# Ignalina/znippy

Hardware: AMD Instinct MI355X
Metric: decompress MB/s (uncompressed) + compress MB/s, 100k x 10KB archive (higher is better)
Workload: dtype u8; 1 GPU; 100k x 10KiB text chunks (BASELINE configs[1]); rows_per_gpu=100000, chunk_bytes=10240, bytes_per_gpu=1024000000, blob_bytes_per_gpu=6400000, parallelism=row-cursor ranges x1, pipelining=step k+1 queued before step k's counters are read (two runs in flight)

## Files before the change

### znippy_amd/csrc/api.hip

```cpp
#include <unistd.h>
#include "common.h"
#include "encode.h"
#include "../../include/znippy_hip.h"
#include "host/enc_plan.h"
#include "host/gz_plan.h"
#include "host/range_plan.h"
#include "host/rows_plan.h"
#include "host/run_overlap.h"

#include <algorithm>
#include <cstdio>
#include <cstdlib>
#include <cstring>
#include <chrono>
#include <memory>
#include <new>
#include <stdexcept>
#include <string>
#include <vector>
#include <unordered_map>

namespace zn {
int measure_b3_pass_ns(int cus, hipStream_t s, float *ns_per_pass_per_simd, float *ghz);
size_t decode_lit_scratch_bytes(int grid);
// ... 64 lines not shown
    uint8_t *enc_prov = nullptr;
    size_t enc_prov_cap = 0;
    uint32_t *enc_seq = nullptr;
    EncTables *enc_tabs = nullptr;
    hipStream_t aux = nullptr;
    hipStream_t copy = nullptr;
    uint8_t *lit_scratch_b = nullptr;
    uint8_t *fz_lit_pool = nullptr;
    unsigned long long *fz_seq_pool = nullptr;
    uint64_t fz_lit_cap = 0, fz_seq_cap = 0;
    uint16_t *bx_fse_pool = nullptr;
    uint16_t *bx_huf_pool = nullptr;
    uint64_t bx_fse_cap = 0, bx_huf_cap = 0;
    uint32_t *rx_pool = nullptr, *rx_chunk = nullptr;
    uint8_t *rx_cdone = nullptr;
    uint64_t rx_cap = 0;
    uint8_t *vs_pool = nullptr;
    uint64_t vs_cap = 0;
    uint8_t *rr_pool[2] = {nullptr, nullptr};
    uint64_t rr_cap[2] = {0, 0};
    hipEvent_t ev_fork = nullptr, ev_join = nullptr, ev_join2 = nullptr;
    std::vector<KTime> ktimes;
    int n_ktimes = 0;
    std::vector<hipEvent_t> event_pool;
    bool ktime_open = false;
    std::vector<std::pair<size_t, void *>> pinned_pool;
    size_t pinned_pool_bytes = 0;
    std::vector<std::pair<size_t, void *>> dev_pool;
    std::unordered_map<void *, size_t> dev_sizes;
    size_t dev_pool_bytes = 0;
    struct : RowsSwitches {
        unsigned lds_pad = 0;
        int store_g = 0;
        bool edbg = false, no_fused_store = false, no_fork_verify = false, no_run_lanes = false, nohash = false, fz_only = false, tdbg = false, no_fuse_hash = false, trace = false, no_pack = false;
        int ktime = 2;
        bool poison = false;
        int poison_byte = 0;
    } sw;
    int poison_hold = 0;
    int cus = 256;
    bool fork_verify = false;
    hipStream_t lane = nullptr;
    hipEvent_t ev_mark = nullptr, lane_join = nullptr;
    hipEvent_t lane_ev[2][2] = {{nullptr, nullptr}, {nullptr, nullptr}};
    unsigned lane_n[2] = {0, 0};
    bool lanes_on = false, main_dirty = true, mark_pending = false;
    struct LaneRun { zn_run_desc d; hipEvent_t ev; bool on_lane, valid; } lane_prev = {}, lane_hist[2][2] = {};
    uint64_t lane_stats[5] = {0, 0, 0, 0, 0};
    int live_tables = 0;
    bool closing = false;
    unsigned long long *clk_buf = nullptr;
    enum Diag { DIAG_FUSED, DIAG_ITEMS, DIAG_FZ, DIAG_GENERAL, DIAG_BX, DIAG_ENCODE, DIAG_N };
    unsigned long long *diag[DIAG_N] = {};
};

static void read_switches(znippy_ctx *ctx) {
    auto on = [](const char *n) { const char *v = getenv(n); return v && *v && *v != '0'; };
    if (const char *e = getenv("ZNIPPY_DBG")) ctx->sw.dbg = atoi(e);
    if (const char *e = getenv("ZNIPPY_LDS_PAD")) ctx->sw.lds_pad = (unsigned)atoi(e);
    ctx->sw.no_block_items = on("ZNIPPY_NO_BLOCK_ITEMS");
    ctx->sw.no_fused_blocks = on("ZNIPPY_NO_FUSED_BLOCKS");
    ctx->sw.ddbg = on("ZNIPPY_DDBG");
    ctx->sw.edbg = on("ZNIPPY_EDBG");
    ctx->sw.no_fused_store = on("ZNIPPY_NO_FUSED_STORE");
    ctx->sw.nohash = on("ZNIPPY_NOHASH");
    ctx->sw.no_roles = on("ZNIPPY_NO_ROLES");
    ctx->sw.no_fz = on("ZNIPPY_NO_FZ");
    ctx->sw.tdbg = on("ZNIPPY_TDBG");
    ctx->sw.trace = on("ZNIPPY_TRACE");
    ctx->sw.no_lean = on("ZNIPPY_NO_LEAN");
    ctx->sw.no_fork_verify = on("ZNIPPY_NO_FORK_VERIFY");
    ctx->sw.no_run_lanes = on("ZNIPPY_NO_RUN_LANES");
    ctx->sw.no_pack = on("ZNIPPY_NO_PACK");
    if (const char *e = getenv("ZNIPPY_STORE_G")) ctx->sw.store_g = atoi(e) == 1 ? 1 : (atoi(e) == 2 ? 2 : 0);
    ctx->sw.no_stored_only = on("ZNIPPY_NO_STORED_ONLY");
    ctx->sw.no_rx = on("ZNIPPY_NO_RX");
    ctx->sw.no_fuse_hash = on("ZNIPPY_NO_FUSE_HASH");
    ctx->sw.no_bx = on("ZNIPPY_NO_BX");
    if (const char *e = getenv("ZNIPPY_BX_BIG")) { ctx->sw.bx_big = (unsigned)atoi(e); ctx->sw.bx_big_set = true; }
    if (const char *lv = getenv("ZNIPPY_LEVEL")) { const int v = atoi(lv); if (v >= 1 && v <= 22) ctx->level = v; }
    if (const char *wl = getenv("ZNIPPY_WINDOW_LOG")) { const int v = atoi(wl); if (v == 0 || (v >= WINDOW_LOG_MIN && v <= WINDOW_LOG_MAX)) ctx->window_log = v; }
    if (const char *gc = getenv("ZNIPPY_GZ_CUT")) {
        char *end = nullptr;
        const unsigned long long v = strtoull(gc, &end, 10);
        if (*gc >= '0' && *gc <= '9' && end && !*end && gzcut::cut_valid(v)) ctx->gz_cut = v;
    }
    if (const char *bc = getenv("ZNIPPY_BX_CHECKSUM")) { const int v = atoi(bc); if (v == 0 || v == 1) ctx->batch_checksums = v; }
    if (const char *gs = getenv("ZNIPPY_GEN_SHARE")) { const int v = atoi(gs); if (v >= 1 && v <= 4) ctx->gen_share = v; }
    ctx->sw.fz_only = on("ZNIPPY_FZ_ONLY");
    if (const char *e = getenv("ZNIPPY_ROLES_MIN")) ctx->sw.roles_min = (unsigned)atoi(e);
    if (const char *e = getenv("ZNIPPY_KTIME")) ctx->sw.ktime = atoi(e);
    if (const char *e = getenv("ZNIPPY_POISON")) {
        char *end = nullptr;
        const long v = strtol(e, &end, e[0] == '0' && (e[1] == 'x' || e[1] == 'X') ? 16 : 10);
        if (*e && end && !*end && v >= 0 && v <= 255) { ctx->sw.poison = true; ctx->sw.poison_byte = (int)v; }
    }
}

static hipError_t poison_dev(znippy_ctx *ctx, void *p, size_t bytes) {
    if (!p || !bytes) return hipSuccess;
    const hipError_t e = hipMemsetAsync(p, ctx->sw.poison_byte, bytes, ctx->stream);
    return e != hipSuccess ? e : hipStreamSynchronize(ctx->stream);
}

static void *pinned_take(znippy_ctx *ctx, size_t bytes, size_t *cap) {
    size_t best = ctx->pinned_pool.size();
    for (size_t i = 0; i < ctx->pinned_pool.size(); i++)
        if (ctx->pinned_pool[i].first >= bytes && ctx->pinned_pool[i].first <= 4 * bytes + 4096 &&
            (best == ctx->pinned_pool.size() || ctx->pinned_pool[i].first < ctx->pinned_pool[best].first))
// ... 2388 lines not shown
    }
    if (!r->d_ldm) {
        std::vector<uint64_t> desc(r->n, LDM_NONE);
        for (const LdmRound &e : r->h_ldm) desc[e.round] = e.desc;
        LdmRound *dl = nullptr;
        uint64_t *dd = nullptr;
        if (tmalloc(ctx, &dl, sizeof(LdmRound) * r->h_ldm.size()) != hipSuccess || tmalloc(ctx, &dd, 8 * (size_t)r->n) != hipSuccess ||
            hipMemcpy(dl, r->h_ldm.data(), sizeof(LdmRound) * r->h_ldm.size(), hipMemcpyHostToDevice) != hipSuccess ||
            hipMemcpy(dd, desc.data(), 8 * (size_t)r->n, hipMemcpyHostToDevice) != hipSuccess) {
            (void)hipGetLastError();
            tfree(ctx, dl);
            tfree(ctx, dd);
            return false;
        }
        r->d_ldm = dl; r->d_ldm_desc = dd;
    }
    return true;
}

struct EncRun { const void *d_src; void *d_blob_out; uint64_t blob_cap; unsigned slot; ResSlab res; uint32_t *tree_out; uint32_t align; const uint32_t *pad; };
static_assert(ENC_HIGH_TIER_LEVEL == HIGH_TIER_LEVEL, "host/enc_plan.h restates the tier boundary of encode.h");

static EncShape rounds_shape(const znippy_rounds *r) {
    return EncShape{r->n, r->n_items, r->n_small, r->n_wide, r->in_bytes, r->enc_bytes, r->fuse_tiles, r->plan.n_tiles, r->n_tree_entries, r->ldm_entries,
                    r->store_incompressible, r->emit_tree, r->blob_align};
}
static EncodeArgs rounds_encode_args(znippy_ctx *ctx, const znippy_rounds *r, const EncPlan &p, const EncRun &run) {
    EncodeArgs a{};
    a.items = r->items;
    a.src = (const uint8_t *)run.d_src; a.src_off = r->src_off; a.len = r->len;
    a.prov = ctx->enc_prov; a.seq_scratch = ctx->enc_seq;
    a.piece_len = r->piece_len; a.piece_start = r->piece_start; a.tabs = ctx->enc_tabs;
    a.high = p.high;
    a.tail_mark = p.tail_mark;
    a.window_log = p.window_log;
    if (p.far) { a.ldm = ctx->ldm; a.ldm_desc = r->d_ldm_desc; }
    if (ctx->sw.edbg)
        a.dbg = diag_cycle<8>(ctx, znippy_ctx::DIAG_ENCODE, ctx->stream, nullptr, [](const unsigned long long *h) {
            if (h[0]) fprintf(stderr, "[znippy edbg] wide blocks=%llu  cycles per block: setup=%.0f matching=%.0f literals=%.0f sequences=%.0f\n", h[0],
                              (double)h[1] / h[0], (double)h[2] / h[0], (double)h[3] / h[0], (double)h[4] / h[0]);
        });
    return a;
}
static GatherArgs rounds_gather_args(znippy_ctx *ctx, const znippy_rounds *r, const EncPlan &p, const EncRun &run) {
    GatherArgs g{};
    g.items = r->items; g.n_pieces = r->n_items; g.piece_len = r->piece_len; g.piece_start = r->piece_start;
    g.local_excl = r->local_excl; g.block_tot = r->block_tot; g.prov = ctx->enc_prov;
    g.src = (const uint8_t *)run.d_src; g.src_off = r->src_off;
    g.blob_out = (uint8_t *)run.d_blob_out; g.blob_cap = run.blob_cap;
    g.blob_offset = run.res.blob_offset(); g.blob_size = run.res.blob_size(); g.total = run.res.total(); g.overflow = run.res.overflow();
    g.stored = p.store_decide ? r->stored : nullptr;
    g.skip_stored_copy = p.fuse_store ? 1 : 0;
    g.pad = run.pad;
    g.small_pieces = p.small_pieces ? 1 : 0;
    return g;
}

static int enc_clear(znippy_ctx *ctx, znippy_rounds *r, const EncPlan &, const EncRun &run) {
    hipStream_t s = ctx->stream;
    if (r->run_seq >= 2) HIPCHK(ctx, hipStreamWaitEvent(s, r->ev_res[run.slot], 0));
    HIPCHK(ctx, hipMemsetAsync(run.res.base, 0, ResSlab::clear_bytes(r->n), s));
    HIPCHK(ctx, hipMemsetAsync(ctx->cursor, 0, 64, s));
    HIPCHK(ctx, hipEventRecord(ctx->ev_fork, s));
    return ZNIPPY_OK;
}

static int enc_far_index(znippy_ctx *ctx, znippy_rounds *r, const EncPlan &p, const EncRun &run) {
    if (!p.far) return ZNIPPY_OK;
    ktime_begin(ctx, "ldm_index");
    HIPCHK(ctx, hipMemsetAsync(ctx->ldm, 0xFF, 4 * r->ldm_entries, ctx->stream));
    launch_ldm_index(r->d_ldm, (uint32_t)r->h_ldm.size(), r->ldm_chunks, (const uint8_t *)run.d_src, r->src_off, r->len, ctx->ldm, ctx->stream);
    ktime_end(ctx);
    return ZNIPPY_OK;
// ... 46 lines not shown
}

static void enc_gather(znippy_ctx *ctx, znippy_rounds *r, const EncPlan &p, const EncRun &run) {
    const GatherArgs g = rounds_gather_args(ctx, r, p, run);
    timed(ctx, "gather", ctx->stream, [&] { launch_gather(g, ctx->stream); });
}

static int enc_hash_store(znippy_ctx *ctx, znippy_rounds *r, const EncPlan &p, const EncRun &run) {
    if (p.fuse_store) return hash_rounds_async(ctx, r, run.res, run.d_src, nullptr, run.d_blob_out, run.blob_cap, run.align, run.tree_out);
    if (p.fork_aux) HIPCHK(ctx, hipStreamWaitEvent(ctx->stream, ctx->ev_join, 0));
    return ZNIPPY_OK;
}

static int enc_results_out(znippy_ctx *ctx, znippy_rounds *r, const EncPlan &, const EncRun &run) {
    HIPCHK(ctx, hipEventRecord(r->ev_enc[run.slot], ctx->stream));
    HIPCHK(ctx, hipStreamWaitEvent(ctx->copy, r->ev_enc[run.slot], 0));
    const uint32_t n16 = (uint32_t)((r->res_bytes + 15) / 16);
    hipLaunchKernelGGL(k_results_out, dim3(std::min<uint32_t>((n16 + 255) / 256, 8)), dim3(256), 0, ctx->copy,
                       reinterpret_cast<uint4 *>(r->h_res_m[run.slot]), reinterpret_cast<const uint4 *>(run.res.base), n16);
    if (run.tree_out) {
        const uint32_t t16 = 2 * r->n_tree_entries;
        hipLaunchKernelGGL(k_results_out, dim3(std::min<uint32_t>((t16 + 255) / 256, 8)), dim3(256), 0, ctx->copy,
                           reinterpret_cast<uint4 *>(r->h_tree_m[run.slot]), reinterpret_cast<const uint4 *>(run.tree_out), t16);
    }
    HIPCHK(ctx, hipEventRecord(r->ev_res[run.slot], ctx->copy));
    return ZNIPPY_OK;
}

static int rounds_launch(znippy_ctx *ctx, znippy_rounds *r, const void *d_src, void *d_blob_out, uint64_t blob_cap, unsigned slot, bool *queued) {
    ctx->n_ktimes = 0;
    if (!r->n) return ZNIPPY_OK;
    int rc = ensure_encoder(ctx);
    if (rc) return rc;
    EncEnv env{ctx->level, ctx->window_log, ctx->encode_grid, ctx->encode_grid_small, (bool)ctx->sw.nohash, (bool)ctx->sw.no_fuse_hash, (bool)ctx->sw.no_fused_store, false};
    env.ldm_ok = enc_window_log(env) && ensure_ldm(ctx, r);
    if (r->prov_bytes + 64 > ctx->enc_prov_cap) {
        HIPCHK(ctx, hipStreamSynchronize(ctx->stream));
        if (ctx->enc_prov) (void)hipFree(ctx->enc_prov);
        ctx->enc_prov = nullptr; ctx->enc_prov_cap = 0;
        HIPCHK(ctx, hipMalloc(&ctx->enc_prov, r->prov_bytes + 64));
        ctx->enc_prov_cap = r->prov_bytes + 64;
        if (ctx->sw.poison) HIPCHK(ctx, poison_dev(ctx, ctx->enc_prov, ctx->enc_prov_cap));
    }
    const EncPlan p = enc_plan(rounds_shape(r), env);
    const EncRun run{d_src, d_blob_out, blob_cap, slot, r->dev(slot), p.tree_out ? r->tree_m[slot] : nullptr, r->blob_align, p.pad ? r->piece_pad : nullptr};
    *queued = true;
    if ((rc = enc_clear(ctx, r, p, run)) || (rc = enc_far_index(ctx, r, p, run))) return rc;
    enc_blocks(ctx, r, p, run);
    if ((rc = enc_hash_beside(ctx, r, p, run))) return rc;
    enc_layout(ctx, r, p, run);
    enc_gather(ctx, r, p, run);
    if ((rc = enc_hash_store(ctx, r, p, run)) || (rc = enc_results_out(ctx, r, p, run))) return rc;
    HIPCHK(ctx, hipGetLastError());
    r->tree_run[slot] = p.emit_tree;
    r->slot = slot;
    r->run_seq++;
    return ZNIPPY_OK;
}

static void rounds_abandon(znippy_ctx *ctx, znippy_rounds *r, unsigned slot) {
    if (hipEventRecord(ctx->ev_join, ctx->aux) == hipSuccess) (void)hipStreamWaitEvent(ctx->stream, ctx->ev_join, 0);
    (void)hipStreamWaitEvent(ctx->copy, r->ev_enc[slot], 0);
    (void)hipStreamSynchronize(ctx->stream);
    (void)hipStreamSynchronize(ctx->copy);
    (void)hipGetLastError();
}
static int rounds_queue(znippy_ctx *ctx, znippy_rounds *r, const void *d_src, void *d_blob_out, uint64_t blob_cap) {
// ... 997 lines not shown
```

### znippy_amd/csrc/encode.h

```cpp
#pragma once
#include "common.h"
#include <cstring>
#include <vector>

namespace zn {

constexpr uint32_t BLOCK_BYTES = 128 * 1024;
constexpr uint32_t HDR_ROOM = 16;
constexpr uint32_t MAX_SEQ = 16384;
constexpr uint32_t SKIP_PIECE = 64u << 10;

struct FseSymTT {
    int32_t delta_find_state;
    uint32_t delta_nb_bits;
};

struct EncTables {
    uint16_t ll_state[64], ml_state[64], of_state[32];
    FseSymTT ll_tt[36], ml_tt[53], of_tt[29];
};

constexpr uint32_t ITEM_SKIP = 1, ITEM_FIRST = 2;

struct EncItem {
    uint32_t round;
    uint32_t block;
    uint32_t n_blocks;
    uint32_t flags;
    uint64_t prov;
};

__host__ __device__ inline uint64_t enc_slot_bytes(uint32_t n) { return ((HDR_ROOM + 16 + 2ull * n + (n >> 2) + 64) + 15) & ~15ull; }

struct EncodeArgs {
    const EncItem *items;
    const uint32_t *order;
    uint32_t n_items;
    const uint32_t *n_items_dev;
    unsigned long long *dbg;
    uint32_t *retry_list, *retry_count;
    uint32_t *cursor;
    uint32_t batch;
    const uint8_t *src;
    const uint64_t *src_off, *len;
    uint8_t *prov;
    uint32_t *seq_scratch;
    uint32_t *piece_len;
    uint64_t *piece_start;
    const EncTables *tabs;
    int tail_mark;
    int high;
    int fuse_tiles;
    HashArgs h;
    int window_log;
    const uint32_t *ldm;
    const uint64_t *ldm_desc;
};

constexpr uint64_t LDM_NONE = 0;
constexpr uint32_t LDM_MIN_LOG = 11, LDM_MAX_LOG = 22;
constexpr uint64_t LDM_MAX_ENTRIES = 1ull << 27;
constexpr uint32_t LDM_CHUNK = 16384;
constexpr int WINDOW_LOG_MIN = 17, WINDOW_LOG_MAX = 27;
struct LdmRound {
    uint32_t round;
    uint32_t first_chunk;
    uint64_t desc;
};
__host__ __device__ inline uint32_t ldm_log2(uint64_t len) {
    uint32_t l = LDM_MIN_LOG;
    while (l < LDM_MAX_LOG && (1ull << l) * 64 < len) l++;
    return l;
}

struct GatherArgs {
    const EncItem *items;
    uint32_t n_pieces;
    const uint32_t *piece_len;
    const uint64_t *piece_start;
    const uint64_t *local_excl, *block_tot;
    const uint8_t *prov, *src;
    const uint64_t *src_off;
    uint8_t *blob_out;
    uint64_t blob_cap;
// ... 22 lines not shown
```

### znippy_amd/csrc/host/enc_plan.cc

```cpp
#include "enc_plan.h"

#include <algorithm>

int enc_window_log(const EncEnv &e) {
    return e.level >= ENC_HIGH_TIER_LEVEL ? e.window_log : 0;
}

static EncLaunch enc_share(const EncShape &s, uint32_t n_items, int g) {
    EncLaunch l{};
    l.on = n_items != 0;
    if (!l.on) return l;
    l.n_items = n_items;
    l.use_order = !(n_items == s.n_items);
    l.batch = std::max<uint32_t>(1, std::min<uint32_t>(16, n_items / (uint32_t)(g * 2)));
    l.grid = std::min<int>(g, (int)n_items);
    return l;
}

EncPlan enc_plan(const EncShape &s, const EncEnv &e) {
    EncPlan p{};
    p.high = e.level >= ENC_HIGH_TIER_LEVEL;
    p.window_log = enc_window_log(e);
    p.tail_mark = p.high && !p.window_log;
    p.far = p.window_log && s.ldm_entries && e.ldm_ok;
    p.store_decide = s.store_incompressible;
    p.pad = s.blob_align > 1;
    p.emit_tree = s.emit_tree && !e.nohash;
    p.tree_out = p.emit_tree && s.n_tree_entries;
    p.fuse_hash = s.fuse_tiles && !s.store_incompressible && !e.nohash && !e.no_fuse_hash;
    const bool heavy = s.in_bytes && (s.in_bytes - s.enc_bytes) * 2 >= s.in_bytes;
    p.fuse_store = heavy && !s.store_incompressible &&
                   !e.no_fused_store && !e.nohash;
    p.fork_aux = !p.fuse_store && !p.fuse_hash;
    p.hash_beside = p.fork_aux && !e.nohash;
    p.small_pieces = s.n_items && s.n_wide == 0 && (p.fuse_store || s.in_bytes / s.n_items <= 16384);
    p.wide = enc_share(s, s.n_wide, e.encode_grid);
    p.small = enc_share(s, s.n_small, e.encode_grid_small);
    if (p.small.on && p.fuse_hash)
        p.small.grid = std::min<int>(e.encode_grid_small, (int)((s.plan_n_tiles + s.fuse_tiles - 1) / s.fuse_tiles));
    if (s.n_small) {
        p.retry.on = true;
        p.retry.n_items = s.n_small; p.retry.use_order = true;
        p.retry.batch = 1;
        p.retry.grid = std::min<int>(e.encode_grid, (int)s.n_small);
    }
    return p;
}
```

### znippy_amd/csrc/host/enc_plan.h

```cpp
#pragma once
#include <stddef.h>
#include <stdint.h>

constexpr int ENC_HIGH_TIER_LEVEL = 4;

struct EncShape {
    uint32_t n;
    uint32_t n_items;
    uint32_t n_small, n_wide;
    uint64_t in_bytes, enc_bytes;
    int fuse_tiles;
    uint32_t plan_n_tiles;
    uint32_t n_tree_entries;
    uint64_t ldm_entries;
    bool store_incompressible;
    bool emit_tree;
    uint32_t blob_align;
};

struct EncEnv {
    int level, window_log;
    int encode_grid, encode_grid_small;
    bool nohash, no_fuse_hash, no_fused_store;
    bool ldm_ok;
};

struct EncLaunch {
    bool on;
    uint32_t n_items;
    bool use_order;
    int grid;
    uint32_t batch;
};

struct EncPlan {
    bool high;
    int window_log;
    bool tail_mark;
    bool far;
    bool fuse_hash;
    bool fuse_store;
    bool fork_aux;
    bool hash_beside;
    bool emit_tree;
    bool tree_out;
    bool store_decide;
    bool pad;
    bool small_pieces;
    EncLaunch wide, small, retry;
};

int enc_window_log(const EncEnv &e);
EncPlan enc_plan(const EncShape &s, const EncEnv &e);

struct ResSlab {
    uint8_t *base;
    uint32_t n;
    uint64_t *total() const { return reinterpret_cast<uint64_t *>(base); }
    uint32_t *overflow() const { return reinterpret_cast<uint32_t *>(base + 8); }
    uint64_t *blob_offset() const { return reinterpret_cast<uint64_t *>(base + 16); }
    uint64_t *blob_size() const { return blob_offset() + n; }
    uint32_t *digests() const { return reinterpret_cast<uint32_t *>(base + 16 + 16 * (size_t)n); }
    static size_t clear_bytes(size_t n) { return 16 + 16 * n; }
    static size_t bytes(size_t n) { return 16 + n * (8 + 8 + 32); }
};
```

### znippy_amd/csrc/zstd_encode.hip

```cpp
#include "common.h"
#include "encode.h"
#include "hash_dev.h"

namespace zn {


__device__ __forceinline__ uint32_t ld32(const uint8_t *p) {
    uint32_t v;
    __builtin_memcpy(&v, p, 4);
    return v;
}
__device__ __forceinline__ uint4 ld128(const uint8_t *p) {
    uint4 v;
    __builtin_memcpy(&v, p, 16);
    return v;
}
template <uint32_t HASH_LOG>
__device__ __forceinline__ uint32_t hash4(uint32_t v) { return (v * 2654435761u) >> (32 - HASH_LOG); }
__device__ __forceinline__ int hib(uint32_t v) { return 31 - __clz(v); }

__device__ __forceinline__ bool ldm_anchor(uint32_t v) { return (hash4<22>(v) & 63u) == 0; }
__device__ __forceinline__ uint32_t ldm_key(const uint8_t *p) {
    uint64_t h = 0;
#pragma unroll
// ... 48 lines not shown
        add(1, 1);
        while (n > 0) {
            *p++ = (uint8_t)acc;
            acc >>= 8;
            n = n > 8 ? n - 8 : 0;
        }
        return p;
    }
};

struct CState {
    uint32_t v;
    const uint16_t *st;
    const FseSymTT *tt;
    uint32_t log;
    __device__ __forceinline__ void init(const uint16_t *st_, const FseSymTT *tt_, uint32_t log_, uint32_t sym) {
        st = st_; tt = tt_; log = log_;
        const FseSymTT t = tt[sym];
        uint32_t nb = (t.delta_nb_bits + (1u << 15)) >> 16;
        uint32_t val = (nb << 16) - t.delta_nb_bits;
        v = st[(int32_t)(val >> nb) + t.delta_find_state];
    }
    __device__ __forceinline__ void encode(BitW &b, uint32_t sym) {
        const FseSymTT t = tt[sym];
        uint32_t nb = (v + t.delta_nb_bits) >> 16;
        b.add(v, nb);
        v = st[(int32_t)(v >> nb) + t.delta_find_state];
    }
    __device__ __forceinline__ void flush(BitW &b) { b.add(v, log); }
};

constexpr uint32_t SMALL_BLOCK = 16 * 1024;
constexpr uint32_t SMALL_MAX_SEQ = SMALL_BLOCK / 40;

template <uint32_t HASH_LOG>
struct EncShared {
    uint16_t table[1u << HASH_LOG];
    EncTables tabs;
    uint32_t seqs[HASH_LOG == 11 ? 3 * (SMALL_MAX_SEQ + 1) : 4];
    uint32_t sink[64];
};

__device__ __forceinline__ void wave_copy(uint8_t *dst, const uint8_t *src, uint32_t n, uint32_t lane) {
    if (n < 128) {
        for (uint32_t i = lane; i < n; i += 64) dst[i] = src[i];
        return;
    }
    const uint32_t head = (uint32_t)((16 - ((uintptr_t)dst & 15)) & 15);
    if (lane < head) dst[lane] = src[lane];
    const uint32_t body = (n - head) >> 4;
    for (uint32_t i = lane; i < body; i += 64) {
        uint4 v = ld128(src + head + (size_t)i * 16);
        *reinterpret_cast<uint4 *>(dst + head + (size_t)i * 16) = v;
    }
    const uint32_t done = head + body * 16;
    if (done + lane < n) dst[done + lane] = src[done + lane];
}

__device__ __forceinline__ uint32_t suni(uint32_t v) { return (uint32_t)__builtin_amdgcn_readfirstlane((int)v); }
__device__ __forceinline__ uint32_t rdlane(uint32_t v, uint32_t l) { return (uint32_t)__builtin_amdgcn_readlane((int)v, (int)l); }

template <class SH>
__device__ __noinline__ uint8_t *encode_sequences(SH &S, const uint32_t *seqs, uint32_t nseq, uint8_t *p, uint32_t lane, uint32_t ov_bias) {
    uint32_t *const ebits = reinterpret_cast<uint32_t *>(S.table);
    const uint32_t st_ll = S.tabs.ll_state[lane & 63], st_ml = S.tabs.ml_state[lane & 63], st_of = S.tabs.of_state[lane & 31];
    for (uint32_t i = lane; i < 200; i += 64) ebits[i] = 0;
    uint32_t vl = 0, vm = 0, vo = 0;
    uint32_t bitpos = 0;
    for (uint32_t e0 = 0; e0 < nseq; e0 += 64) {
        const uint32_t cnt = nseq - e0 < 64 ? nseq - e0 : 64;
        const bool on = lane < cnt;
        const uint32_t i = nseq - 1 - (e0 + (on ? lane : 0));
        const uint32_t ll = seqs[3 * i], mlb = seqs[3 * i + 1], ov = seqs[3 * i + 2] + ov_bias;
        const uint32_t lc = ll < 64 ? c_ll_code[ll] : (uint32_t)hib(ll) + 19;
        const uint32_t mc = mlb < 128 ? c_ml_code[mlb] : (uint32_t)hib(mlb) + 36;
        const uint32_t oc = (uint32_t)hib(ov);
        const FseSymTT tl = S.tabs.ll_tt[lc], tm = S.tabs.ml_tt[mc], to = S.tabs.of_tt[oc];
        uint32_t f_l = 0, f_m = 0, f_o = 0;
        for (uint32_t j = 0; j < cnt; j++) {
            const uint32_t dl = rdlane(tl.delta_nb_bits, j), fl = rdlane((uint32_t)tl.delta_find_state, j);
            const uint32_t dm = rdlane(tm.delta_nb_bits, j), fm = rdlane((uint32_t)tm.delta_find_state, j);
            const uint32_t d_o = rdlane(to.delta_nb_bits, j), fo = rdlane((uint32_t)to.delta_find_state, j);
            if (e0 + j == 0) {
                uint32_t nb = (dm + (1u << 15)) >> 16;
                vm = rdlane(st_ml, (uint32_t)((int32_t)(((nb << 16) - dm) >> nb) + (int32_t)fm));
                nb = (d_o + (1u << 15)) >> 16;
                vo = rdlane(st_of, (uint32_t)((int32_t)(((nb << 16) - d_o) >> nb) + (int32_t)fo));
                nb = (dl + (1u << 15)) >> 16;
                vl = rdlane(st_ll, (uint32_t)((int32_t)(((nb << 16) - dl) >> nb) + (int32_t)fl));
            } else {
                uint32_t nb = (vo + d_o) >> 16;
// ... 731 lines not shown
    else if (n <= 16383 && comp <= 16383) { sf = 2; hdr = 4; }
    else { sf = 3; hdr = 5; }
    if (hdr + comp + (n >> 6) >= 3 + n || (nstreams == 4 && (ssz[0] > 65535 || ssz[1] > 65535 || ssz[2] > 65535))) return 0;
    asm volatile("s_waitcnt vmcnt(0)" ::: "memory");
    if (lane == 0) {
        const uint32_t nb = sf == 0 ? 10u : (sf == 2 ? 14u : 18u);
        const uint64_t h = 2ull | ((uint64_t)sf << 2) | ((uint64_t)n << 4) | ((uint64_t)comp << (4 + nb));
        for (uint32_t k = 0; k < hdr; k++) dst[k] = (uint8_t)(h >> (8 * k));
        if (direct) dst[hdr] = (uint8_t)(127 + last);
    }
    if (direct) {
        const uint32_t nbytes = (last + 1) / 2;
        for (uint32_t i = lane; i < nbytes; i += 64) {
            const uint32_t la = codes[2 * i] >> 16, lb = (2 * i + 1 < last) ? codes[2 * i + 1] >> 16 : 0;
            const uint32_t wa = la ? L + 1 - la : 0, wb = lb ? L + 1 - lb : 0;
            dst[hdr + 1 + i] = (uint8_t)((wa << 4) | wb);
        }
    } else {
        for (uint32_t i = lane; i < tree_bytes; i += 64) dst[hdr + i] = wbuf[i];
    }
    uint8_t *d = dst + hdr + tree_bytes;
    if (nstreams == 4) {
        if (lane == 0) {
            d[0] = (uint8_t)ssz[0]; d[1] = (uint8_t)(ssz[0] >> 8);
            d[2] = (uint8_t)ssz[1]; d[3] = (uint8_t)(ssz[1] >> 8);
            d[4] = (uint8_t)ssz[2]; d[5] = (uint8_t)(ssz[2] >> 8);
        }
        d += 6;
    }
    wave_copy(d, tmp, streams_bytes, lane);
    return hdr + comp;
}

template <uint32_t HASH_LOG, bool HIGH = false, bool WIN = false>
__global__ __launch_bounds__(64) void k_zstd_encode(EncodeArgs a) {
    constexpr uint32_t HASH_SIZE = 1u << HASH_LOG;
    __shared__ __attribute__((aligned(16))) EncShared<HASH_LOG> S;
    __shared__ uint32_t s_item, s_raw;
    const uint32_t lane = threadIdx.x;
    if (a.n_items_dev && *a.n_items_dev == 0) return;
    {
        const uint32_t *g = reinterpret_cast<const uint32_t *>(a.tabs);
        uint32_t *l = reinterpret_cast<uint32_t *>(&S.tabs);
        for (uint32_t i = lane; i < sizeof(EncTables) / 4; i += 64) l[i] = g[i];
    }
    uint32_t *const seqs = HASH_LOG == 11 ? S.seqs : a.seq_scratch + (size_t)blockIdx.x * MAX_SEQ * 3;

    uint32_t next = 0, lim = 0, first = 0;
    const uint32_t n_items = a.n_items_dev ? *a.n_items_dev : a.n_items;
    uint32_t d_round = 0, d_block = 0, d_nblocks = 0, d_flags = ITEM_SKIP, d_id = 0;
    uint64_t d_prov = 0, d_rlen = 0, d_soff = 0;
    for (;;) {
        if (next == lim) {
            __syncthreads();
            uint32_t batch = a.batch;
            if (HASH_LOG == 11 && !HIGH && a.fuse_tiles) {
                const uint32_t FUSE_TILES = (uint32_t)a.fuse_tiles;
                if (lane == 0) s_item = atomicAdd(a.cursor, FUSE_TILES);
                __syncthreads();
                const uint32_t t0 = s_item;
                if (t0 >= a.h.n_tiles) break;
                uint32_t r_first = 0, r_end = 0;
                for (uint32_t k = 0; k < FUSE_TILES && t0 + k < a.h.n_tiles; k++) {
                    const Tile t = a.h.tiles[t0 + k];
                    hash_tile<false>(a.h, t);
                    if (k == 0) r_first = t.first_unit;
                    r_end = t.first_unit + t.n_units;
                }
                next = first = r_first;
                batch = r_end - r_first;
                lim = r_end;
            } else {
                if (lane == 0) s_item = atomicAdd(a.cursor, a.batch);
                __syncthreads();
                next = first = s_item;
                lim = next + a.batch;
            }
            const uint32_t mine = first + lane;
            d_flags = ITEM_SKIP;
            if (lane < batch && mine < n_items) {
                d_id = a.order ? a.order[mine] : mine;
                const EncItem e = a.items[d_id];
                d_round = e.round; d_block = e.block; d_nblocks = e.n_blocks; d_flags = e.flags; d_prov = e.prov;
                d_rlen = a.len[e.round];
                d_soff = a.src_off[e.round];
            }
        }
        const uint32_t item = next++;
        if (item >= n_items) break;
        __syncthreads();
        const uint32_t bl = item - first;
        EncItem it;
        it.round = __shfl(d_round, bl); it.block = __shfl(d_block, bl); it.n_blocks = __shfl(d_nblocks, bl);
        it.flags = __shfl(d_flags, bl); it.prov = __shfl(d_prov, bl);
        const uint32_t item_id = __shfl(d_id, bl);
        if (it.flags & ITEM_SKIP) continue;
        const uint64_t rlen = __shfl(d_rlen, bl);
        const uint8_t *const rsrc = a.src + __shfl(d_soff, bl);
        const uint64_t boff = (uint64_t)it.block * BLOCK_BYTES;
        const uint32_t n = (uint32_t)((rlen - boff) < BLOCK_BYTES ? (rlen - boff) : BLOCK_BYTES);
        const uint8_t *const in = rsrc + boff;
        const bool last = it.block + 1 == it.n_blocks;
        uint8_t *const blk = a.prov + it.prov + HDR_ROOM;
        uint8_t *const lits = blk + 3 + 3;
        const uint32_t seq_div = HASH_LOG == 13 ? 8u : 40u;
        const uint32_t max_seq = (n / seq_div) < MAX_SEQ ? (n / seq_div) : MAX_SEQ;
        for (uint32_t o = lane * 128; o + 4 <= n; o += 64 * 128)
            __builtin_amdgcn_global_load_lds((const __attribute__((address_space(1))) void *)(in + o),
                                             (__attribute__((address_space(3))) void *)S.sink, 4, 0, 0);
        unsigned long long t_last = (HASH_LOG == 13 && a.dbg) ? __builtin_amdgcn_s_memtime() : 0;
#define ESTAMP(i) do { if (HASH_LOG == 13 && a.dbg && lane == 0) { const unsigned long long now_ = __builtin_amdgcn_s_memtime(); atomicAdd(&a.dbg[i], now_ - t_last); t_last = now_; } } while (0)
        if (HASH_LOG == 13 && a.dbg && lane == 0) atomicAdd(&a.dbg[0], 1ull);
        {
            uint4 *t4 = reinterpret_cast<uint4 *>(S.table);
            const uint4 ones = make_uint4(~0u, ~0u, ~0u, ~0u);
            for (uint32_t i = lane; i < HASH_SIZE / 8; i += 64) t4[i] = ones;
        }
        __syncthreads();
        ESTAMP(1);
        const uint32_t PRE = WIN ? suni((uint32_t)(boff < (1ull << a.window_log) ? boff : (1ull << a.window_log))) : 0u;
        const uint8_t *const inb = in - PRE;
        const uint32_t nq = n + PRE;
        uint32_t nseq = 0, lit_total = 0;
        uint32_t anchor = PRE;
        uint32_t emitted = PRE;
        uint32_t base = PRE, misses = 0;
        bool gave_up = false;
        const uint32_t scan_end = nq >= 8 ? nq - 7 : 0;
        if constexpr (HIGH) {
            constexpr uint32_t LMAX = 64;
            uint4 *const B = reinterpret_cast<uint4 *>(S.table);
            uint32_t r0 = 0, r1 = 0, r2 = 0;
            uint64_t ldm_slot = 0;
            uint32_t ldm_mask = 0, far_dmax = 0;
            bool far_on = false;
            if constexpr (WIN) {
                constexpr uint32_t NEAR = 64u << 10;
                const uint32_t p0 = PRE > NEAR ? PRE - NEAR : 0u;
                for (uint32_t b0 = p0; b0 < PRE; b0 += 256) {
                    const uint32_t p = b0 + 4 * lane;
                    if (p < PRE && p + 4 <= nq) {
                        const uint32_t h = hash4<10>(ld32(inb + p));
                        const uint4 b = B[h];
                        B[h] = make_uint4((b.x << 16) | (p & 0xFFFFu), (b.y << 16) | (b.x >> 16), (b.z << 16) | (b.y >> 16), (b.w << 16) | (b.z >> 16));
                    }
                }
                const uint64_t desc = a.ldm ? a.ldm_desc[it.round] : LDM_NONE;
                far_on = desc != LDM_NONE;
                ldm_slot = desc & ((1ull << 48) - 1);
                ldm_mask = (1u << (uint32_t)(desc >> 48)) - 1u;
                far_dmax = 1u << a.window_log;
            }
// ... 330 lines not shown
                        if (partial) {
                            const uint32_t fl = __ffsll((unsigned long long)partial) - 1;
                            ml += fl * 16 + __shfl(good[q], fl);
                            done = true;
                        } else {
                            ml += 1024;
                        }
                    }
                    if (done) break;
                }
                    }
                    const uint32_t ll = mpos - anchor;
                    if (emitted < mpos) {
                        if (emitted < base) {
                            wave_copy(lits + lit_total + (emitted - anchor), inb + emitted, base - emitted, lane);
                            emitted = base;
                        }
                        if (pos >= emitted && pos < mpos) lits[lit_total + (pos - anchor)] = (uint8_t)v;
                    }
                    if (lane == 0) {
                        seqs[3 * nseq] = ll;
                        seqs[3 * nseq + 1] = ml - 3;
                        seqs[3 * nseq + 2] = mpos - mcand;
                    }
                    lit_total += ll;
                    nseq++;
                    anchor = mpos + ml;
                    emitted = anchor;
                }
                store_tail();
                base = anchor > base + 64 ? anchor : base + 64;
            }
        } else {
            while (base < scan_end && nseq < max_seq) {
                const uint32_t pos = base + lane;
                uint32_t cand = 0, hitf = 0;
                if (pos < scan_end) {
                    const uint32_t v = ld32(inb + pos);
                    const uint32_t h = hash4<HASH_LOG>(v);
                    const uint32_t e = S.table[h];
                    S.table[h] = (uint16_t)pos;
                    if (e != 0xFFFF) {
                        uint32_t c = (pos & ~0xFFFFu) | e;
                        if (c >= pos) c -= 0x10000u;
                        if (c < pos && pos >= PRE && ld32(inb + c) == v) { cand = c; hitf = 1; }
                    }
                }
                const uint64_t hit = __ballot(hitf != 0);
                if (!hit) {
                    misses++;
                    base += 64 * (1 + (misses >> 4 > 7 ? 7 : misses >> 4));
                    continue;
                }
                misses = 0;
                const uint32_t win = __ffsll((unsigned long long)hit) - 1;
                const uint32_t mpos = __shfl(pos, win), mcand = __shfl(cand, win);
                uint32_t ml = 4;
                for (;;) {
                    uint32_t good[4];
    #pragma unroll
                    for (int q = 0; q < 4; q++) {
                        const uint32_t o = ml + q * 1024 + lane * 16;
                        uint32_t g = 0;
                        if (mpos + o + 16 <= nq) {
                            uint4 x = ld128(inb + mpos + o), y = ld128(inb + mcand + o);
                            const uint32_t d0 = x.x ^ y.x, d1 = x.y ^ y.y, d2 = x.z ^ y.z, d3 = x.w ^ y.w;
                            g = 16;
                            if (d0 | d1 | d2 | d3) {
                                if (d0) g = (__ffs(d0) - 1) >> 3;
                                else if (d1) g = 4 + ((__ffs(d1) - 1) >> 3);
                                else if (d2) g = 8 + ((__ffs(d2) - 1) >> 3);
                                else g = 12 + ((__ffs(d3) - 1) >> 3);
                            }
                        } else {
                            while (g < 16 && mpos + o + g < nq && inb[mpos + o + g] == inb[mcand + o + g]) g++;
                        }
                        good[q] = g;
                    }
                    bool done = false;
    #pragma unroll
                    for (int q = 0; q < 4; q++) {
                        if (done) break;
                        const uint64_t partial = __ballot(good[q] != 16);
                        if (partial) {
                            const uint32_t fl = __ffsll((unsigned long long)partial) - 1;
                            ml += fl * 16 + __shfl(good[q], fl);
                            done = true;
                        } else {
                            ml += 1024;
                        }
                    }
                    if (done) break;
                }
                const uint32_t ll = mpos - anchor;
                wave_copy(lits + lit_total, inb + anchor, ll, lane);
                if (lane == 0) {
                    seqs[3 * nseq] = ll;
                    seqs[3 * nseq + 1] = ml - 3;
                    seqs[3 * nseq + 2] = mpos - mcand;
                }
                lit_total += ll;
                nseq++;
                anchor = mpos + ml;
                base = anchor;
            }
        }
        if (HASH_LOG == 11 && a.retry_list &&
            ((nseq >= max_seq && base < scan_end) || (a.high && (nseq > 8 || lit_total + (nq - anchor) >= HUF_MIN_LITS)))) {
            if (lane == 0) a.retry_list[atomicAdd(a.retry_count, 1u)] = item_id;
            continue;
        }
        {
            const uint32_t e0 = (HASH_LOG == 13 && emitted > anchor) ? emitted : anchor;
            if (e0 < nq && !gave_up) wave_copy(lits + lit_total + (e0 - anchor), inb + e0, nq - e0, lane);
        }
        lit_total += nq - anchor;
        __syncthreads();

        ESTAMP(2);
        uint32_t lit_sec = 0;
        if (HIGH && lit_total >= HUF_MIN_LITS && !gave_up)
            lit_sec = huf_literals_any(S, lits, lit_total, lits + ((lit_total + 3) & ~3u), blk + 3, lane);
        else if (HASH_LOG == 13 && lit_total >= HUF_MIN_LITS && !gave_up)
            lit_sec = huf_literals(S, lits, lit_total, lits + ((lit_total + 3) & ~3u), blk + 3, lane);
        ESTAMP(3);
        bool raw = nseq == 0 && lit_sec == 0;
        uint32_t csize = 0;
        if (!raw) {
            if (!lit_sec) {
                if (lane == 0) {
                    blk[3] = (uint8_t)(0 | (3 << 2) | ((lit_total & 15) << 4));
                    blk[4] = (uint8_t)(lit_total >> 4);
                    blk[5] = (uint8_t)(lit_total >> 12);
                }
                lit_sec = 3 + lit_total;
            }
// ... 13 lines not shown
                uint32_t plen = 0;
                if (lane == 0) {
                    BitW b{p + hl + 1, 0, 0};
                    CState sl, so, sm;
                    for (int32_t i = (int32_t)nseq - 1; i >= 0; i--) {
                        const uint32_t ll = seqs[3 * i], mlb = seqs[3 * i + 1], ov = seqs[3 * i + 2] + (HIGH ? 0u : 3u);
                        const uint32_t lc = ll < 64 ? c_ll_code[ll] : (uint32_t)hib(ll) + 19;
                        const uint32_t mc = mlb < 128 ? c_ml_code[mlb] : (uint32_t)hib(mlb) + 36;
                        const uint32_t oc = (uint32_t)hib(ov);
                        if (i == (int32_t)nseq - 1) {
                            sm.init(S.tabs.ml_state, S.tabs.ml_tt, 6, mc);
                            so.init(S.tabs.of_state, S.tabs.of_tt, 5, oc);
                            sl.init(S.tabs.ll_state, S.tabs.ll_tt, 6, lc);
                        } else {
                            so.encode(b, oc);
                            sm.encode(b, mc);
                            sl.encode(b, lc);
                        }
                        b.add(ll - c_ll_base_e[lc], c_ll_bits_e[lc]);
                        b.add(mlb + 3 - c_ml_base_e[mc], c_ml_bits_e[mc]);
                        b.add(ov - (1u << oc), oc);
                    }
                    sm.flush(b);
                    so.flush(b);
                    sl.flush(b);
                    plen = (uint32_t)(b.close() - p);
                }
                p += suni(plen);
            }
            csize = (uint32_t)(p - (blk + 3));
            if (csize >= n) raw = true;
        }
        ESTAMP(4);
        const bool tail_mark = a.tail_mark && last && it.n_blocks > 1;
        if (lane == 0) {
            uint32_t piece_len = 0, hdr_len = 0;
            const uint32_t last_bit = last && !tail_mark ? 1u : 0u;
            if (!raw) {
                const uint32_t bh = last_bit | (2u << 1) | (csize << 3);
                blk[0] = (uint8_t)bh; blk[1] = (uint8_t)(bh >> 8); blk[2] = (uint8_t)(bh >> 16);
                piece_len = 3 + csize;
            }
            if (raw) {
                const uint32_t bh = last_bit | (0u << 1) | (n << 3);
                blk[0] = (uint8_t)bh; blk[1] = (uint8_t)(bh >> 8); blk[2] = (uint8_t)(bh >> 16);
                piece_len = 3 + n;
            }
            if (tail_mark) piece_len += 3;
            if (it.block == 0) {
                uint8_t h[16];
                uint32_t k = 0;
                h[k++] = 0x28; h[k++] = 0xB5; h[k++] = 0x2F; h[k++] = 0xFD;
                if (rlen < 256) { h[k++] = 0x20; h[k++] = (uint8_t)rlen; }
                else if (rlen < 65792) { h[k++] = 0x60; uint32_t v = (uint32_t)rlen - 256; h[k++] = (uint8_t)v; h[k++] = (uint8_t)(v >> 8); }
                else if (rlen <= 0xFFFFFFFFull) { h[k++] = 0xA0; for (int i = 0; i < 4; i++) h[k++] = (uint8_t)(rlen >> (8 * i)); }
                else { h[k++] = 0xE0; for (int i = 0; i < 8; i++) h[k++] = (uint8_t)(rlen >> (8 * i)); }
                hdr_len = k;
                for (uint32_t i = 0; i < k; i++) blk[(int32_t)i - (int32_t)k] = h[i];
            }
            s_raw = raw ? 1u : 0u;
            a.piece_len[item_id] = piece_len + hdr_len;
            a.piece_start[item_id] = it.prov + HDR_ROOM - hdr_len;
        }
        __syncthreads();
        if (s_raw) wave_copy(blk + 3, in, n, lane);
        if (tail_mark && lane == 0) {
            uint8_t *const t = blk + 3 + (s_raw ? n : csize);
            t[0] = 1; t[1] = 0; t[2] = 0;
        }
    }
}

template <bool PAD>
__global__ __launch_bounds__(256) void k_piece_scan(const uint32_t *piece_len, const uint32_t *pad, uint32_t n, uint64_t *local_excl,
                                                    uint64_t *block_tot) {
    __shared__ uint64_t wsum[4];
    const uint32_t i = blockIdx.x * 256 + threadIdx.x, lane = threadIdx.x & 63, w = threadIdx.x >> 6;
    uint64_t v = i < n ? piece_len[i] : 0;
    if (PAD && i < n) v += pad[i];
    uint64_t inc = v;
#pragma unroll
    for (int d = 1; d < 64; d <<= 1) {
        uint64_t y = __shfl_up(inc, d);
        if (lane >= (uint32_t)d) inc += y;
    }
    if (lane == 63) wsum[w] = inc;
    __syncthreads();
    uint64_t wbase = 0;
    for (uint32_t k = 0; k < w; k++) wbase += wsum[k];
    if (i < n) local_excl[i] = wbase + inc - v;
    if (threadIdx.x == 255) block_tot[blockIdx.x] = wbase + inc;
}

__device__ __forceinline__ void wave_zero(uint8_t *dst, uint32_t n, uint32_t lane) {
    uint32_t head = (uint32_t)((16 - ((uintptr_t)dst & 15)) & 15);
    if (head > n) head = n;
    if (lane < head) dst[lane] = 0;
    const uint32_t body = (n - head) >> 4;
    for (uint32_t i = lane; i < body; i += 64) *reinterpret_cast<uint4 *>(dst + head + (size_t)i * 16) = make_uint4(0, 0, 0, 0);
    const uint32_t done = head + body * 16;
    if (done + lane < n) dst[done + lane] = 0;
}
// ... 284 lines not shown
```

Baseline: 2.216 million MB/s.

## Reuse wave-held head words for candidate checks and literal copies in small-row encoder

New measurement: 2.215 million MB/s, median of 2. No clear change (-0.0%).

```diff
diff --git a/znippy_amd/csrc/api.hip b/znippy_amd/csrc/api.hip
--- a/znippy_amd/csrc/api.hip
+++ b/znippy_amd/csrc/api.hip
@@ -120,7 +120,7 @@
     struct : RowsSwitches {
         unsigned lds_pad = 0;
         int store_g = 0;
-        bool edbg = false, no_fused_store = false, no_fork_verify = false, no_run_lanes = false, nohash = false, fz_only = false, tdbg = false, no_fuse_hash = false, trace = false, no_pack = false;
+        bool edbg = false, no_fused_store = false, no_fork_verify = false, no_run_lanes = false, nohash = false, fz_only = false, tdbg = false, no_fuse_hash = false, trace = false, no_pack = false, no_enc_heads = false;
         int ktime = 2;
         bool poison = false;
         int poison_byte = 0;
@@ -163,6 +163,7 @@
     if (const char *e = getenv("ZNIPPY_STORE_G")) ctx->sw.store_g = atoi(e) == 1 ? 1 : (atoi(e) == 2 ? 2 : 0);
     ctx->sw.no_stored_only = on("ZNIPPY_NO_STORED_ONLY");
     ctx->sw.no_rx = on("ZNIPPY_NO_RX");
+    ctx->sw.no_enc_heads = on("ZNIPPY_NO_ENC_HEADS");
     ctx->sw.no_fuse_hash = on("ZNIPPY_NO_FUSE_HASH");
     ctx->sw.no_bx = on("ZNIPPY_NO_BX");
     if (const char *e = getenv("ZNIPPY_BX_BIG")) { ctx->sw.bx_big = (unsigned)atoi(e); ctx->sw.bx_big_set = true; }
@@ -2617,13 +2618,19 @@
     a.prov = ctx->enc_prov; a.seq_scratch = ctx->enc_seq;
     a.piece_len = r->piece_len; a.piece_start = r->piece_start; a.tabs = ctx->enc_tabs;
     a.high = p.high;
+    a.heads = p.enc_heads;
     a.tail_mark = p.tail_mark;
     a.window_log = p.window_log;
     if (p.far) { a.ldm = ctx->ldm; a.ldm_desc = r->d_ldm_desc; }
     if (ctx->sw.edbg)
-        a.dbg = diag_cycle<8>(ctx, znippy_ctx::DIAG_ENCODE, ctx->stream, nullptr, [](const unsigned long long *h) {
+        a.dbg = diag_cycle<EDBG_WORDS>(ctx, znippy_ctx::DIAG_ENCODE, ctx->stream, nullptr, [](const unsigned long long *h) {
             if (h[0]) fprintf(stderr, "[znippy edbg] wide blocks=%llu  cycles per block: setup=%.0f matching=%.0f literals=%.0f sequences=%.0f\n", h[0],
                               (double)h[1] / h[0], (double)h[2] / h[0], (double)h[3] / h[0], (double)h[4] / h[0]);
+            unsigned long long t[EDBG_SLOTS] = {};
+            for (uint32_t c = 0; c < EDBG_COPIES; c++)
+                for (uint32_t i = 0; i < EDBG_SLOTS; i++) t[i] += h[EDBG_SMALL + c * EDBG_SLOTS + i];
+            if (t[0]) fprintf(stderr, "[znippy edbg] small rows=%llu  cycles per row: dequeue=%.0f tile-hash=%.0f setup=%.0f window-scan=%.0f extension=%.0f literal-copy=%.0f sequences=%.0f bookkeeping=%.0f\n", t[0],
+                              (double)t[1] / t[0], (double)t[2] / t[0], (double)t[3] / t[0], (double)t[4] / t[0], (double)t[5] / t[0], (double)t[6] / t[0], (double)t[7] / t[0], (double)t[8] / t[0]);
         });
     return a;
 }
@@ -2736,7 +2743,7 @@
     if (!r->n) return ZNIPPY_OK;
     int rc = ensure_encoder(ctx);
     if (rc) return rc;
-    EncEnv env{ctx->level, ctx->window_log, ctx->encode_grid, ctx->encode_grid_small, (bool)ctx->sw.nohash, (bool)ctx->sw.no_fuse_hash, (bool)ctx->sw.no_fused_store, false};
+    EncEnv env{ctx->level, ctx->window_log, ctx->encode_grid, ctx->encode_grid_small, (bool)ctx->sw.nohash, (bool)ctx->sw.no_fuse_hash, (bool)ctx->sw.no_fused_store, false, (bool)ctx->sw.no_enc_heads};
     env.ldm_ok = enc_window_log(env) && ensure_ldm(ctx, r);
     if (r->prov_bytes + 64 > ctx->enc_prov_cap) {
         HIPCHK(ctx, hipStreamSynchronize(ctx->stream));
diff --git a/znippy_amd/csrc/encode.h b/znippy_amd/csrc/encode.h
--- a/znippy_amd/csrc/encode.h
+++ b/znippy_amd/csrc/encode.h
@@ -21,6 +21,8 @@
 };
 
 constexpr uint32_t ITEM_SKIP = 1, ITEM_FIRST = 2;
+
+constexpr uint32_t EDBG_SMALL = 8, EDBG_SLOTS = 16, EDBG_COPIES = 64, EDBG_WORDS = EDBG_SMALL + EDBG_SLOTS * EDBG_COPIES;
 
 struct EncItem {
     uint32_t round;
@@ -50,6 +52,7 @@
     const EncTables *tabs;
     int tail_mark;
     int high;
+    int heads;
     int fuse_tiles;
     HashArgs h;
     int window_log;
diff --git a/znippy_amd/csrc/host/enc_plan.cc b/znippy_amd/csrc/host/enc_plan.cc
--- a/znippy_amd/csrc/host/enc_plan.cc
+++ b/znippy_amd/csrc/host/enc_plan.cc
@@ -25,6 +25,7 @@
     p.far = p.window_log && s.ldm_entries && e.ldm_ok;
     p.store_decide = s.store_incompressible;
     p.pad = s.blob_align > 1;
+    p.enc_heads = !e.no_enc_heads;
     p.emit_tree = s.emit_tree && !e.nohash;
     p.tree_out = p.emit_tree && s.n_tree_entries;
     p.fuse_hash = s.fuse_tiles && !s.store_incompressible && !e.nohash && !e.no_fuse_hash;
diff --git a/znippy_amd/csrc/host/enc_plan.h b/znippy_amd/csrc/host/enc_plan.h
--- a/znippy_amd/csrc/host/enc_plan.h
+++ b/znippy_amd/csrc/host/enc_plan.h
@@ -23,6 +23,7 @@
     int encode_grid, encode_grid_small;
     bool nohash, no_fuse_hash, no_fused_store;
     bool ldm_ok;
+    bool no_enc_heads;
 };
 
 struct EncLaunch {
@@ -47,6 +48,7 @@
     bool store_decide;
     bool pad;
     bool small_pieces;
+    bool enc_heads;
     EncLaunch wide, small, retry;
 };
 
diff --git a/znippy_amd/csrc/zstd_encode.hip b/znippy_amd/csrc/zstd_encode.hip
--- a/znippy_amd/csrc/zstd_encode.hip
+++ b/znippy_amd/csrc/zstd_encode.hip
@@ -104,6 +104,10 @@
 
 constexpr uint32_t SMALL_BLOCK = 16 * 1024;
 constexpr uint32_t SMALL_MAX_SEQ = SMALL_BLOCK / 40;
+#ifndef ZN_EXT_SMALL
+#define ZN_EXT_SMALL 4
+#endif
+constexpr int EXT_SMALL = ZN_EXT_SMALL;
 
 template <uint32_t HASH_LOG>
 struct EncShared {
@@ -129,6 +133,10 @@
     if (done + lane < n) dst[done + lane] = src[done + lane];
 }
 
+__device__ __forceinline__ void lds_fence() {
+    asm volatile("s_waitcnt lgkmcnt(0)" ::: "memory");
+    __builtin_amdgcn_wave_barrier();
+}
 __device__ __forceinline__ uint32_t suni(uint32_t v) { return (uint32_t)__builtin_amdgcn_readfirstlane((int)v); }
 __device__ __forceinline__ uint32_t rdlane(uint32_t v, uint32_t l) { return (uint32_t)__builtin_amdgcn_readlane((int)v, (int)l); }
 
@@ -926,6 +934,69 @@
     return hdr + comp;
 }
 
+template <int EXT>
+__device__ __forceinline__ uint32_t extend_small(const uint8_t *inu, uint32_t mpos, uint32_t mcand, uint32_t nq, uint32_t lane) {
+    auto first_diff = [](const uint4 &x, const uint4 &y, uint32_t sh) -> uint32_t {
+        uint32_t d0 = x.x ^ y.x, d1 = x.y ^ y.y, d2 = x.z ^ y.z, d3 = x.w ^ y.w;
+        if (sh) {
+            d0 = sh >= 4 ? 0u : d0 & (~0u << (8 * sh));
+            d1 = sh >= 8 ? 0u : (sh > 4 ? d1 & (~0u << (8 * (sh - 4))) : d1);
+            d2 = sh >= 12 ? 0u : (sh > 8 ? d2 & (~0u << (8 * (sh - 8))) : d2);
+            d3 = sh > 12 ? d3 & (~0u << (8 * (sh - 12))) : d3;
+        }
+        uint32_t g = 16;
+        if (d0 | d1 | d2 | d3) {
+            if (d0) g = (__ffs(d0) - 1) >> 3;
+            else if (d1) g = 4 + ((__ffs(d1) - 1) >> 3);
+            else if (d2) g = 8 + ((__ffs(d2) - 1) >> 3);
+            else g = 12 + ((__ffs(d3) - 1) >> 3);
+        }
+        return g;
+    };
+    uint32_t ml = 4;
+    for (;;) {
+        const uint32_t rem = nq - mpos - ml;
+        if (rem < 16 && mcand + ml < 16) {
+            while (mpos + ml < nq && inu[mpos + ml] == inu[mcand + ml]) ml++;
+            return ml;
+        }
+        const uint32_t nw = (rem >> 10) < (uint32_t)EXT ? (rem >> 10) : (uint32_t)EXT;
+        const uint32_t o0 = ml + lane * 16;
+        uint4 x[EXT > 0 ? EXT : 1], y[EXT > 0 ? EXT : 1];
+#pragma unroll
+        for (int q = 0; q < EXT; q++)
+            if ((uint32_t)q < nw) { x[q] = ld128(inu + (mpos + o0 + q * 1024)); y[q] = ld128(inu + (mcand + o0 + q * 1024)); }
+        const bool tail = EXT == 0 || nw < (uint32_t)EXT;
+        const uint32_t ot = o0 + nw * 1024;
+        const int32_t left = (int32_t)(nq - mpos) - (int32_t)ot;
+        const uint32_t sh = left >= 16 ? 0u : (left > 0 ? 16u - (uint32_t)left : 0u);
+        uint4 xt = make_uint4(0, 0, 0, 0), yt = xt;
+        if (tail) { xt = ld128(inu + (left > 0 ? mpos + ot - sh : 0u)); yt = ld128(inu + (left > 0 ? mcand + ot - sh : 0u)); }
+        bool done = false;
+#pragma unroll
+        for (int q = 0; q < EXT; q++) {
+            if (done || (uint32_t)q >= nw) continue;
+            const uint32_t g = first_diff(x[q], y[q], 0);
+            const uint64_t partial = __ballot(g != 16);
+            if (partial) {
+                const uint32_t fl = __ffsll((unsigned long long)partial) - 1;
+                ml += fl * 16 + rdlane(g, fl);
+                done = true;
+            } else {
+                ml += 1024;
+            }
+        }
+        if (done) return ml;
+        if (tail) {
+            const uint32_t g = left > 0 ? first_diff(xt, yt, sh) - sh : 0u;
+            const uint64_t partial = __ballot(g != 16);
+            if (EXT == 0 && !partial) { ml += 1024; continue; }
+            const uint32_t fl = __ffsll((unsigned long long)partial) - 1;
+            return ml + fl * 16 + rdlane(g, fl);
+        }
+    }
+}
+
 template <uint32_t HASH_LOG, bool HIGH = false, bool WIN = false>
 __global__ __launch_bounds__(64) void k_zstd_encode(EncodeArgs a) {
     constexpr uint32_t HASH_SIZE = 1u << HASH_LOG;
@@ -939,6 +1010,9 @@
         for (uint32_t i = lane; i < sizeof(EncTables) / 4; i += 64) l[i] = g[i];
     }
     uint32_t *const seqs = HASH_LOG == 11 ? S.seqs : a.seq_scratch + (size_t)blockIdx.x * MAX_SEQ * 3;
+    unsigned long long t_s = (HASH_LOG == 11 && a.dbg) ? __builtin_amdgcn_s_memtime() : 0;
+#define SSTAMP(i) do { if (HASH_LOG == 11 && a.dbg) { const unsigned long long now_ = __builtin_amdgcn_s_memtime(); \
+        if (lane == 0) atomicAdd(&a.dbg[EDBG_SMALL + (blockIdx.x & (EDBG_COPIES - 1)) * EDBG_SLOTS + (i)], now_ - t_s); t_s = now_; } } while (0)
 
     uint32_t next = 0, lim = 0, first = 0;
     const uint32_t n_items = a.n_items_dev ? *a.n_items_dev : a.n_items;
@@ -954,6 +1028,7 @@
                 __syncthreads();
                 const uint32_t t0 = s_item;
                 if (t0 >= a.h.n_tiles) break;
+                SSTAMP(1);
                 uint32_t r_first = 0, r_end = 0;
                 for (uint32_t k = 0; k < FUSE_TILES && t0 + k < a.h.n_tiles; k++) {
                     const Tile t = a.h.tiles[t0 + k];
@@ -964,11 +1039,13 @@
                 next = first = r_first;
                 batch = r_end - r_first;
                 lim = r_end;
+                SSTAMP(2);
             } else {
                 if (lane == 0) s_item = atomicAdd(a.cursor, a.batch);
                 __syncthreads();
                 next = first = s_item;
                 lim = next + a.batch;
+                SSTAMP(1);
             }
             const uint32_t mine = first + lane;
             d_flags = ITEM_SKIP;
@@ -1005,13 +1082,16 @@
         unsigned long long t_last = (HASH_LOG == 13 && a.dbg) ? __builtin_amdgcn_s_memtime() : 0;
 #define ESTAMP(i) do { if (HASH_LOG == 13 && a.dbg && lane == 0) { const unsigned long long now_ = __builtin_amdgcn_s_memtime(); atomicAdd(&a.dbg[i], now_ - t_last); t_last = now_; } } while (0)
         if (HASH_LOG == 13 && a.dbg && lane == 0) atomicAdd(&a.dbg[0], 1ull);
+        if (HASH_LOG == 11 && a.dbg && lane == 0) atomicAdd(&a.dbg[EDBG_SMALL + (blockIdx.x & (EDBG_COPIES - 1)) * EDBG_SLOTS], 1ull);
         {
             uint4 *t4 = reinterpret_cast<uint4 *>(S.table);
             const uint4 ones = make_uint4(~0u, ~0u, ~0u, ~0u);
             for (uint32_t i = lane; i < HASH_SIZE / 8; i += 64) t4[i] = ones;
         }
-        __syncthreads();
+        if (HASH_LOG == 11) lds_fence();
+        else __syncthreads();
         ESTAMP(1);
+        SSTAMP(3);
         const uint32_t PRE = WIN ? suni((uint32_t)(boff < (1ull << a.window_log) ? boff : (1ull << a.window_log))) : 0u;
         const uint8_t *const inb = in - PRE;
         const uint32_t nq = n + PRE;
@@ -1408,68 +1488,54 @@
                 base = anchor > base + 64 ? anchor : base + 64;
             }
         } else {
+            const bool heads = a.heads != 0;
+            const bool hand_early = a.high && a.retry_list;
+            uint32_t pv = 0, pbase = 0xFFFFFFFFu;
             while (base < scan_end && nseq < max_seq) {
+                if (hand_early && (nseq > 8 || lit_total >= HUF_MIN_LITS)) break;
                 const uint32_t pos = base + lane;
-                uint32_t cand = 0, hitf = 0;
+                uint32_t cand = 0, hitf = 0, v = 0, c = 0;
+                bool probe = false;
                 if (pos < scan_end) {
-                    const uint32_t v = ld32(inb + pos);
+                    v = ld32(inb + pos);
                     const uint32_t h = hash4<HASH_LOG>(v);
                     const uint32_t e = S.table[h];
                     S.table[h] = (uint16_t)pos;
                     if (e != 0xFFFF) {
-                        uint32_t c = (pos & ~0xFFFFu) | e;
+                        c = (pos & ~0xFFFFu) | e;
                         if (c >= pos) c -= 0x10000u;
-                        if (c < pos && pos >= PRE && ld32(inb + c) == v) { cand = c; hitf = 1; }
+                        probe = c < pos && pos >= PRE;
                     }
                 }
+                if (heads) {
+                    const uint32_t near = (uint32_t)__shfl((int)pv, (int)((c - pbase) & 63u));
+                    if (probe) {
+                        const uint32_t cv = (c >= pbase && c - pbase < 64) ? near : ld32(inb + c);
+                        if (cv == v) { cand = c; hitf = 1; }
+                    }
+                } else if (probe && ld32(inb + c) == v) { cand = c; hitf = 1; }
                 const uint64_t hit = __ballot(hitf != 0);
+                SSTAMP(4);
                 if (!hit) {
                     misses++;
+                    pv = v; pbase = base;
                     base += 64 * (1 + (misses >> 4 > 7 ? 7 : misses >> 4));
                     continue;
                 }
                 misses = 0;
                 const uint32_t win = __ffsll((unsigned long long)hit) - 1;
-                const uint32_t mpos = __shfl(pos, win), mcand = __shfl(cand, win);
-                uint32_t ml = 4;
-                for (;;) {
-                    uint32_t good[4];
-    #pragma unroll
-                    for (int q = 0; q < 4; q++) {
-                        const uint32_t o = ml + q * 1024 + lane * 16;
-                        uint32_t g = 0;
-                        if (mpos + o + 16 <= nq) {
-                            uint4 x = ld128(inb + mpos + o), y = ld128(inb + mcand + o);
-                            const uint32_t d0 = x.x ^ y.x, d1 = x.y ^ y.y, d2 = x.z ^ y.z, d3 = x.w ^ y.w;
-                            g = 16;
-                            if (d0 | d1 | d2 | d3) {
-                                if (d0) g = (__ffs(d0) - 1) >> 3;
-                                else if (d1) g = 4 + ((__ffs(d1) - 1) >> 3);
-                                else if (d2) g = 8 + ((__ffs(d2) - 1) >> 3);
-                                else g = 12 + ((__ffs(d3) - 1) >> 3);
-                            }
-                        } else {
-                            while (g < 16 && mpos + o + g < nq && inb[mpos + o + g] == inb[mcand + o + g]) g++;
-                        }
-                        good[q] = g;
-                    }
-                    bool done = false;
-    #pragma unroll
-                    for (int q = 0; q < 4; q++) {
-                        if (done) break;
-                        const uint64_t partial = __ballot(good[q] != 16);
-                        if (partial) {
-                            const uint32_t fl = __ffsll((unsigned long long)partial) - 1;
-                            ml += fl * 16 + __shfl(good[q], fl);
-                            done = true;
-                        } else {
-                            ml += 1024;
-                        }
-                    }
-                    if (done) break;
-                }
+                const uint32_t mpos = base + win, mcand = rdlane(cand, win);
+                const uint64_t inoff = (uint64_t)(inb - a.src);
+                const uint8_t *const inu = a.src + (((uint64_t)suni((uint32_t)(inoff >> 32)) << 32) | suni((uint32_t)inoff));
+                const uint32_t ml = extend_small<EXT_SMALL>(inu, mpos, mcand, nq, lane);
+                SSTAMP(5);
                 const uint32_t ll = mpos - anchor;
-                wave_copy(lits + lit_total, inb + anchor, ll, lane);
+                if (heads && (anchor >= base || (anchor >= pbase && pbase + 64 >= base))) {
+                    const uint32_t ppos = pbase + lane;
+                    if (anchor < base && ppos >= anchor && ppos < base) lits[lit_total + (ppos - anchor)] = (uint8_t)pv;
+                    if (pos >= anchor && pos < mpos) lits[lit_total + (pos - anchor)] = (uint8_t)v;
+                } else wave_copy(lits + lit_total, inb + anchor, ll, lane);
+                SSTAMP(6);
                 if (lane == 0) {
                     seqs[3 * nseq] = ll;
                     seqs[3 * nseq + 1] = ml - 3;
@@ -1478,6 +1544,7 @@
                 lit_total += ll;
                 nseq++;
                 anchor = mpos + ml;
+                pv = v; pbase = base;
                 base = anchor;
             }
         }
@@ -1557,6 +1624,7 @@
             if (csize >= n) raw = true;
         }
         ESTAMP(4);
+        SSTAMP(7);
         const bool tail_mark = a.tail_mark && last && it.n_blocks > 1;
         if (lane == 0) {
             uint32_t piece_len = 0, hdr_len = 0;
@@ -1593,6 +1661,7 @@
             uint8_t *const t = blk + 3 + (s_raw ? n : csize);
             t[0] = 1; t[1] = 0; t[2] = 0;
         }
+        SSTAMP(8);
     }
 }
 
```
